# cvxgrp/qcqp

Hardware: AMD Instinct MI355X
Metric: restarts x coord-sweeps / sec (improve COORD_DESCENT phase-2 sweeps, 2n^2 flops each; whole step timed) (higher is better)
Workload: dtype f64

## Files before the change

### qcqp_amd/csrc/cd_life.hip

```cpp
#include "cd_life.h"

#include <cstdio>
#include <cstdlib>

#include "onevar.h"
#include "cd_phase1_sep.h"
#include "cd_chain.h"
#include "cd_roles.h"

namespace qcqpmi {
namespace {

constexpr int L2_WD = 1 << 21;
enum { L2_ABORT = 3 };

__device__ __attribute__((always_inline)) inline RqOwn l2_own(int NB, int CS, int m, int NMW) {
    RqOwn o;
    const int rest = NB - CS;
    o.NB = NB;
    if (m < 0) { o.first = rest; o.stride = 1; o.nu = CS; }
    else { o.first = m; o.stride = NMW; o.nu = m < rest ? (rest - m + NMW - 1) / NMW : 0; }
    return o;
}

// ... 982 lines not shown
                    if (l2_tl(sid, ct, TD)[cc] < 0) for (int64_t j = tid; j < n16; j += NT) Xg[j * 16 + cc] = 0.0;
                    continue;
                }
                if (!lf_generate) {
                    const int id = l2_tl(sid, ct, TD)[cc];
                    GLB const double *src = glb(a0.b.X) + ((int64_t)(id >> 4) * n16) * 16 + (id & 15);
                    for (int64_t j0 = tid; j0 < n16; j0 += 4 * NT) {
                        double t4[4];
#pragma unroll
                        for (int u = 0; u < 4; u++) t4[u] = (j0 + u * NT < n16) ? src[(j0 + u * NT) * 16] : 0.0;
#pragma unroll
                        for (int u = 0; u < 4; u++) if (j0 + u * NT < n16) Xg[(j0 + u * NT) * 16 + cc] = t4[u];
                    }
                }
            }
            if (lf_generate) {
                if (tid == 0) {
                    int cnt = 0;
                    for (int k = 0; k < NS; k++) if (l2_tl(snew, k >> 4, TD)[k & 15]) p1cols[cnt++] = k;
                    ctl[4] = cnt; ctl[5] = 0;
                }
                __syncthreads();
                const int ncolg = ctl[4], nchg = (int)((n16 + 127) / 128);
                for (;;) {
                    int ch = 0;
                    if (lane == 0) ch = atomicAdd(&ctl[5], 1);
                    ch = __builtin_amdgcn_readfirstlane(ch);
                    if (ch >= ncolg * nchg) break;
                    const int c = p1cols[ch / nchg], ct = c >> 4, cc = c & 15;
                    GLB double *Xg = Xg0 + (int64_t)ct * n16 * 16;
                    const int64_t j = (int64_t)(ch % nchg) * 128 + 2 * lane;
                    const uint64_t sd = l2_tl(sseed, ct, TD)[cc], gidx = l2_tl(sfirst, ct, TD)[cc] + (uint64_t)l2_tl(sid, ct, TD)[cc];
                    if (j < n16) {
                        double xo = 0.0;
                        const double xe = (j < P.n) ? keyed_normal_pair(sd, gidx, (uint64_t)j, &xo) : 0.0;
                        Xg[j * 16 + cc] = xe;
                        Xg[(j + 1) * 16 + cc] = (j + 1 < P.n) ? xo : 0.0;
                    }
                }
            }
            __syncthreads();
            if (lf->prof && tid == 0) atomicAdd((unsigned long long *)lf->prof + 4, (unsigned long long)((long long)__builtin_amdgcn_s_memtime() - pt0));
            if (lf_phase1) {
                const bool band2 = !MULTI && cq == 0.0 && rel == RELOP_EQ && cp > 1e-4 && cr < -1e-3;
                const int cw = band2 ? 128 : 64;
                const int nch = (int)((P.n + cw - 1) / cw);
                for (int64_t t = 0; t < a.num_iters; t++) {
                    if (tid == 0) {
                        int cnt = 0;
                        for (int k = 0; k < NS; k++) if (l2_tl(snew, k >> 4, TD)[k & 15] && !l2_tl(p1fin, k >> 4, TD)[k & 15]) p1cols[cnt++] = k;
                        ctl[4] = cnt; ctl[5] = 0;
                    }
                    if (tid < NS) { l2_tl(p1key, tid >> 4, TD)[tid & 15] = ordered_key(-QM_INF); l2_tl(p1upd, tid >> 4, TD)[tid & 15] = 0; }
                    __syncthreads();
                    const int ncol1 = ctl[4];
                    if (ncol1 == 0) break;
                    for (;;) {
                        int ch = 0;
                        if (lane == 0) ch = atomicAdd(&ctl[5], 1);
                        ch = __builtin_amdgcn_readfirstlane(ch);
                        if (ch >= ncol1 * nch) break;
                        const int c = p1cols[ch / nch], ct = c >> 4, cc = c & 15;
                        GLB double *Xg = Xg0 + (int64_t)ct * n16 * 16;
                        const uint64_t sd = l2_tl(sseed, ct, TD)[cc], gidx = l2_tl(sfirst, ct, TD)[cc] + (uint64_t)l2_tl(sid, ct, TD)[cc];
                        double va = -QM_INF;
                        int fl = 0;
                        if (band2) {
                            const int64_t i2[2] = {(int64_t)(ch % nch) * 128 + lane, (int64_t)(ch % nch) * 128 + 64 + lane};
                            const bool on2[2] = {i2[0] < P.n, i2[1] < P.n};
                            double x2[2] = {on2[0] ? Xg[i2[0] * 16 + cc] : 1.0, on2[1] ? Xg[i2[1] * 16 + cc] : 1.0};
                            P1Visit V2[2];
                            p1_band_visit_n<2>(cp, cq, cr, i2, x2, on2, a.tol, lf_viol_tol, sd, gidx, t, V2);
#pragma unroll
                            for (int k = 0; k < 2; k++)
                                if (on2[k]) {
                                    if (V2[k].moved) { Xg[i2[k] * 16 + cc] = x2[k]; fl |= 1; }
                                    if (V2[k].status) fl |= (-V2[k].status) << 8;
                                    va = V2[k].vafter > va ? V2[k].vafter : va;
                                }
                        } else {
                            const int64_t i = (int64_t)(ch % nch) * 64 + lane;
                            if (i < P.n) {
                                if (MULTI) {
                                    double xi = Xg[i * 16 + cc];
                                    P1Visit V;
                                    p1_sep_visit<MAXC>(P, i, xi, a.tol, lf_viol_tol, sd, gidx, t, V);
                                    fl = (V.moved ? 1 : 0) | ((-V.status) << 8);
                                    va = V.vafter;
                                    if (V.moved) Xg[i * 16 + cc] = xi;
                                } else {
                                    const double xi = p1_class_visit(cp, cq, cr, rel, i, Xg[i * 16 + cc], a.tol, lf_viol_tol, sd, gidx, t, &fl, &va);
                                    if (fl & 1) Xg[i * 16 + cc] = xi;
                                }
                            }
                        }
                        const double vmax = wave_max(va);
                        const bool anyupd = __builtin_amdgcn_ballot_w64((fl & 1) != 0) != 0ull;
                        const int st = (fl >> 8) ? -(fl >> 8) : 0;
                        if (lane == 0) { atomicMax(&l2_tl(p1key, ct, TD)[cc], ordered_key(vmax)); if (anyupd) l2_tl(p1upd, ct, TD)[cc] = 1; }
                        if (st) l2_tl(p1st, ct, TD)[cc] = st;
                    }
                    __syncthreads();
                    if (tid < NS && l2_tl(snew, tid >> 4, TD)[tid & 15] && !l2_tl(p1fin, tid >> 4, TD)[tid & 15]) {
                        const int st = tid >> 4, sc = tid & 15;
                        l2_tl(p1sw, st, TD)[sc]++;
                        if (ordered_unkey(l2_tl(p1key, st, TD)[sc]) < lf_viol_tol || !l2_tl(p1upd, st, TD)[sc]) l2_tl(p1fin, st, TD)[sc] = 1;
                    }
                    __syncthreads();
                }
            }
            if (lf->prof && tid == 0) atomicAdd((unsigned long long *)lf->prof + 17, (unsigned long long)((long long)__builtin_amdgcn_s_memtime() - pt0));
            if (tid < NS) l2_tl(p1key, tid >> 4, TD)[tid & 15] = ordered_key(-QM_INF);
            __syncthreads();
            for (int c = 0; c < NS; c++) {
                const int ct = c >> 4, cc = c & 15;
                if (lf_pre || !l2_tl(snew, ct, TD)[cc]) continue;
                GLB const double *Xg = Xg0 + (int64_t)ct * n16 * 16;
                double v = -QM_INF;
                for (int64_t i = tid; i < P.n; i += NT) {
                    const double x = Xg[i * 16 + cc];
                    if (MULTI) {
                        for (int e = P.cptr[i]; e < P.cptr[i + 1]; e++) {
                            const double f = (P.cp[e] * x + P.cq[e]) * x + P.cr[e];
                            const double w = viol_of(f, P.crel[e]);
                            v = w > v ? w : v;
                        }
                    } else {
                        const double f = (cp * x + cq) * x + cr;
                        const double w = (rel == RELOP_EQ) ? fabs(f) : (f > 0.0 ? f : 0.0);
                        v = w > v ? w : v;
                    }
                }
                v = wave_max(v);
                if (lane == 0) atomicMax(&l2_tl(p1key, ct, TD)[cc], ordered_key(v));
            }
            __syncthreads();
            if (tid < NS && l2_tl(snew, tid >> 4, TD)[tid & 15]) {
                const int st = tid >> 4, sc = tid & 15;
                double mvx;
                if (lf_pre) {
                    const int id = l2_tl(sid, st, TD)[sc];
                    mvx = glb(lf->preslack)[id];
                    l2_tl(p1sw, st, TD)[sc] = (int)glb(lf->sweeps1)[id];
                    l2_tl(p1st, st, TD)[sc] = glb(lf->status1)[id];
                    l2_tl(gatep, st, TD)[sc] = glb(lf->ran2)[id];
                } else {
                    mvx = ordered_unkey(l2_tl(p1key, st, TD)[sc]);
                    l2_tl(gatep, st, TD)[sc] = (mvx < lf_viol_tol && l2_tl(p1st, st, TD)[sc] == 0) ? 1 : 0;
                }
                l2_tl(slk, st, TD)[sc] = mvx;
                L2_STORE_SETS(st, sc, mvx)
            }
            __syncthreads();
            if (nlast < 16) {
                for (int w = tid; w < NS * (16 - nlast); w += NT) {
                    const int c = w % NS, ct = c >> 4, cc = c & 15, row = w / NS;
                    if (l2_tl(snew, ct, TD)[cc] || l2_tl(sid, ct, TD)[cc] < 0) {
                        const int nn = l2_tl(TC.n, ct, TD)[cc];
                        double xp = 0.0;
                        if (BK == L2_KIND_BAND) xp = nn >= 2 ? l2_tl(TC.lo, ct, TD)[16 * KCLV + cc] : 0.0;
                        else if (BK == L2_KIND_GEN) xp = nn >= 1 ? l2_tl(TC.hi, ct, TD)[cc] : 0.0;
                        else xp = nn >= 2 ? l2_tl(TC.hi, ct, TD)[16 * KCLV + cc] : l2_tl(TC.hi, ct, TD)[cc];
                        if (!(xp == xp) || __builtin_isinf(xp)) xp = 0.0;
                        (Xg0 + (int64_t)ct * n16 * 16)[(P.n + row) * 16 + cc] = xp;
                    }
                }
                __syncthreads();
            }
            if (LR) {
                const int r16 = 16 * a0.RB;
                const int y0n = lf_pre ? (int)lf->y0_count : 0;
                GLB const double *y0g = glb(lf->y0);
                for (int w = tid; w < NS * (32 + r16); w += NT) {
                    const int c = w % NS, ct = c >> 4, cc = c & 15, rowz = w / NS;
                    const int id = l2_tl(sid, ct, TD)[cc];
                    if (l2_tl(snew, ct, TD)[cc] || id < 0) {
                        double v = 0.0;
                        if (id >= 0 && id < y0n)
                            v = rowz < 32 ? (Xg0 + (int64_t)ct * n16 * 16)[(16 * (int64_t)(NB - 2) + rowz) * 16 + cc]
                                          : y0g[((int64_t)(id >> 4) * r16 + (rowz - 32)) * 16 + (id & 15)];
                        if (rowz < 32) l2_tl(pend, ct, TD)[rowz * 16 + cc] = v;
                        else l2_tl(ytile, ct, TD)[(rowz - 32) * 16 + cc] = v;
                    }
                }
                __syncthreads();
            }
            if (lf->prof && tid == 0) {
                int nn = 0;
                for (int k = 0; k < NS; k++) nn += l2_tl(snew, k >> 4, TD)[k & 15] ? 1 : 0;
                atomicAdd((unsigned long long *)lf->prof + 0, (unsigned long long)((long long)__builtin_amdgcn_s_memtime() - pt0));
                atomicAdd((unsigned long long *)lf->prof + 2, 1ull);
                atomicAdd((unsigned long long *)lf->prof + 3, (unsigned long long)nn);
            }
            __builtin_amdgcn_s_setprio(0);
        }
        if (role == 0) {
            long long *cs_ = l2_tl(cst, rtile, TD);
            if (l2_tl(snew, rtile, TD)[r]) {
#pragma unroll
                for (int f = 0; f < 6; f++) cs_[f * 64 + lane] = 0;
                const int pass = l2_tl(gatep, rtile, TD)[r];
                bool load = LR != 0;
                if (LR) {
                    GLB const CdLife *lf = glb(lifep);
                    if (lf->prebuilt && l2_tl(sid, rtile, TD)[r] < (int)lf->y0_count) load = false;
                }
                cs_[6 * 64 + lane] = 0;
                cs_[4 * 64 + lane] = (pass && !PRE && !load) ? 0 : 1;
                cs_[7 * 64 + lane] = (pass ? (PRE ? 4 : 0) : 1) | (load ? 8 : 0);
                cs_[8 * 64 + lane] = 0;
            } else if (l2_tl(sid, rtile, TD)[r] < 0) {
                cs_[4 * 64 + lane] = 1; cs_[6 * 64 + lane] = 0;
                cs_[7 * 64 + lane] = 2; cs_[8 * 64 + lane] = 0;
            }
        }
        __syncthreads();
        if (tid == 0 && glb(lifep)->prof) *(long long *)(ctl + 6) = (long long)__builtin_amdgcn_s_memtime();

        if (role > 0) {
            if (LR) l2_mfma_lr_role<NMW>(role - 1, rtile);
            else l2_mfma_role<NMW, CS>(role - 1, rtile);
        } else l2_chain_role<NMW, CS, KIND, TILES, LR>(rtile);

        __syncthreads();
        if (sy[L2_ABORT] || (TILES > 1 && l2_tl((int *)sy, 1, TD)[L2_ABORT])) {
            if (tid == 0) __hip_atomic_store(glb(a0.abort), 1, __ATOMIC_RELAXED, __HIP_MEMORY_SCOPE_AGENT);
            break;
        }
        if (tid == 0 && glb(lifep)->prof)
        {
            const long long now_ = (long long)__builtin_amdgcn_s_memtime();
            atomicAdd((unsigned long long *)glb(lifep)->prof + 5, (unsigned long long)(now_ - *(long long *)(ctl + 6)));
            atomicAdd((unsigned long long *)glb(lifep)->prof + 20, (unsigned long long)(now_ - *(long long *)(ctl + 8)));
        }
        {
            const int e0 = P.cptr[P.krep[0]];
            const double cp = P.cp[e0], cq = P.cq[e0], cr = P.cr[e0];
            const int rel = P.crel[e0];
            if (tid == 0) { int cnt = 0; for (int k = 0; k < NS; k++) if (l2_tl(sfin, k >> 4, TD)[k & 15]) p1cols[cnt++] = k; ctl[4] = cnt; }
            if (tid < NS) l2_tl(p1key, tid >> 4, TD)[tid & 15] = ordered_key(-QM_INF);
            __syncthreads();
            const int nfin = ctl[4];
            const int64_t items = (int64_t)nfin * n16;
            for (int64_t w0 = tid; w0 < items; w0 += (int64_t)NT * 8) {
                double xv8[8];
#pragma unroll
                for (int u = 0; u < 8; u++) {
                    const int64_t w = w0 + (int64_t)NT * u;
                    const int col = p1cols[w < items ? w / n16 : 0];
                    const int64_t i = w % n16;
                    xv8[u] = (w < items && i < P.n) ? (Xg0 + (int64_t)(col >> 4) * n16 * 16)[i * 16 + (col & 15)] : 0.0;
                }
#pragma unroll
                for (int u = 0; u < 8; u++) {
                    const int64_t w = w0 + (int64_t)NT * u;
                    if (w < items) {
                        const int col = p1cols[w / n16], id = l2_tl(sid, col >> 4, TD)[col & 15];
                        const int64_t i = w % n16;
                        glb(a0.b.X)[((int64_t)(id >> 4) * n16 + i) * 16 + (id & 15)] = xv8[u];
                        if (i < P.n) {
                            if (MULTI) {
                                double vv = -QM_INF;
                                for (int e = P.cptr[i]; e < P.cptr[i + 1]; e++) {
                                    const double w_ = viol_of((P.cp[e] * xv8[u] + P.cq[e]) * xv8[u] + P.cr[e], P.crel[e]);
                                    vv = w_ > vv ? w_ : vv;
                                }
                                atomicMax(&l2_tl(p1key, col >> 4, TD)[col & 15], ordered_key(vv));
                            } else {
                                const double f = (cp * xv8[u] + cq) * xv8[u] + cr;
                                const double vv = (rel == RELOP_EQ) ? fabs(f) : (f > 0.0 ? f : 0.0);
                                atomicMax(&l2_tl(p1key, col >> 4, TD)[col & 15], ordered_key(vv));
                            }
                        }
                    }
                }
            }
            __syncthreads();
            if (tid < NS && l2_tl(sfin, tid >> 4, TD)[tid & 15]) {
                const int st = tid >> 4, sc = tid & 15;
                const double mx = ordered_unkey(l2_tl(p1key, st, TD)[sc]);
                const int id = l2_tl(sid, st, TD)[sc];
                glb(a0.b.visits)[id] = l2_tl(ovis, st, TD)[sc]; glb(a0.b.accepted)[id] = l2_tl(oacc, st, TD)[sc]; glb(a0.b.sweeps)[id] = l2_tl(oswp, st, TD)[sc];
                glb(a0.b.status)[id] = l2_tl(ost, st, TD)[sc];
                if (a0.b.f0out) glb(a0.b.f0out)[id] = l2_tl(of0, st, TD)[sc];
                if (a0.b.mvout) glb(a0.b.mvout)[id] = mx;
                GLB const CdLife *lf = glb(lifep);
                glb(lf->sweeps1)[id] = l2_tl(p1sw, st, TD)[sc]; glb(lf->status1)[id] = l2_tl(p1st, st, TD)[sc];
                glb(lf->ran2)[id] = (uint8_t)l2_tl(gatep, st, TD)[sc];
                l2_tl(sid, st, TD)[sc] = -1; l2_tl(sfin, st, TD)[sc] = 0;
            }
            __syncthreads();
        }
    }
    if (tid0 == 0 && lf0->prof) {
        const unsigned long long dtl = (unsigned long long)((long long)__builtin_amdgcn_s_memtime() - life_t0);
        atomicAdd((unsigned long long *)lf0->prof + 1, dtl);
        atomicMax((unsigned long long *)lf0->prof + 16, dtl);
    }
}

#undef L2_STORE_SETS

constexpr int L2P_NT = 256;
__global__ __launch_bounds__(L2P_NT) void cd_life_prep_kernel(DevProblem P, const CdLife *life, double *X, int64_t num_iters, double tol) {
    __shared__ unsigned long long key[16];
    __shared__ int upd[16], st1[16], fin[16], sw[16], nact;
    const int tid = threadIdx.x, s = tid & 15, g = tid >> 4;
    GLB const CdLife *lf = glb(life);
    const int64_t id = (int64_t)blockIdx.x * 16 + s;
    const bool valid = id < lf->Rtotal;
    const int64_t n = P.n, n16 = P.n16;
    GLB double *Xt = glb(X) + (int64_t)blockIdx.x * n16 * 16 + s;
    const double viol_tol = lf->viol_tol;
    uint64_t sd = 0, gidx = 0;
    if (valid) {
        const uint64_t pop = (uint64_t)id / (uint64_t)lf->Rpop, rho = (uint64_t)id % (uint64_t)lf->Rpop;
        sd = lf->seed + pop * lf->seed_stride;
        gidx = lf->first_index + pop * lf->first_stride + rho;
    }
    if (lf->generate && valid) {
        for (int64_t j = 2 * g; j < n16; j += 32) {
            double xo = 0.0;
            const double xe = (j < n) ? keyed_normal_pair(sd, gidx, (uint64_t)j, &xo) : 0.0;
            Xt[16 * j] = xe;
            Xt[16 * (j + 1)] = (j + 1 < n) ? xo : 0.0;
        }
    }
    const int e0 = P.cptr[P.krep[0]];
    const double cp = P.cp[e0], cq = P.cq[e0], cr = P.cr[e0];
    const int rel = P.crel[e0];
    if (tid < 16) { fin[tid] = valid ? 0 : 1; sw[tid] = 0; st1[tid] = 0; }
    if (lf->phase1) {
        const bool band2 = cq == 0.0 && rel == RELOP_EQ && cp > 1e-4 && cr < -1e-3;
        for (int64_t t = 0; t < num_iters; t++) {
            if (tid < 16) { key[tid] = ordered_key(-QM_INF); upd[tid] = 0; }
            __syncthreads();
            if (tid == 0) { int c = 0; for (int k = 0; k < 16; k++) c += fin[k] ? 0 : 1; nact = c; }
            __syncthreads();
            if (nact == 0) break;
            double va = -QM_INF;
            int moved = 0, stv = 0;
            if (!fin[s]) {
                for (int64_t j = 2 * g; j < n; j += 32) {
                    if (band2) {
                        const int64_t i2[2] = {j, j + 1};
                        const bool on2[2] = {true, j + 1 < n};
                        double x2[2] = {Xt[16 * j], on2[1] ? Xt[16 * (j + 1)] : 1.0};
                        P1Visit V2[2];
                        p1_band_visit_n<2>(cp, cq, cr, i2, x2, on2, tol, viol_tol, sd, gidx, t, V2);
#pragma unroll
                        for (int k = 0; k < 2; k++)
                            if (on2[k]) {
                                if (V2[k].moved) { Xt[16 * i2[k]] = x2[k]; moved = 1; }
                                if (V2[k].status) stv = V2[k].status;
                                va = V2[k].vafter > va ? V2[k].vafter : va;
                            }
                    } else {
                        for (int64_t i = j; i < j + 2 && i < n; i++) {
                            int fl = 0;
                            double v = 0.0;
                            const double xi = p1_class_visit(cp, cq, cr, rel, i, Xt[16 * i], tol, viol_tol, sd, gidx, t, &fl, &v);
                            if (fl & 1) { Xt[16 * i] = xi; moved = 1; }
                            if (fl >> 8) stv = -(fl >> 8);
                            va = v > va ? v : va;
                        }
                    }
                }
            }
#pragma unroll
            for (int o = 16; o <= 32; o <<= 1) {
                const double w = __shfl_xor(va, o, 64);
                va = w > va ? w : va;
                moved |= __shfl_xor(moved, o, 64);
            }
            if ((tid & 63) < 16 && !fin[s]) { atomicMax(&key[s], ordered_key(va)); if (moved) upd[s] = 1; }
            if (stv) st1[s] = stv;
            __syncthreads();
            if (tid < 16 && !fin[tid]) {
                sw[tid]++;
                if (ordered_unkey(key[tid]) < viol_tol || !upd[tid]) fin[tid] = 1;
            }
        }
    }
    __syncthreads();
    if (tid < 16) key[tid] = ordered_key(-QM_INF);
    __syncthreads();
    double v = -QM_INF;
    if (valid)
        for (int64_t j = 2 * g; j < n; j += 32)
            for (int64_t i = j; i < j + 2 && i < n; i++) {
                const double x = Xt[16 * i];
                const double f = (cp * x + cq) * x + cr;
                const double w = (rel == RELOP_EQ) ? fabs(f) : (f > 0.0 ? f : 0.0);
                v = w > v ? w : v;
            }
#pragma unroll
    for (int o = 16; o <= 32; o <<= 1) { const double w = __shfl_xor(v, o, 64); v = w > v ? w : v; }
    if ((tid & 63) < 16 && valid) atomicMax(&key[s], ordered_key(v));
    __syncthreads();
    if (tid < 16 && valid) {
        const double mvx = ordered_unkey(key[tid]);
        glb(const_cast<double *>(lf->preslack))[id] = mvx;
        glb(lf->sweeps1)[id] = sw[tid];
        glb(lf->status1)[id] = st1[tid];
        glb(lf->ran2)[id] = (mvx < viol_tol && st1[tid] == 0) ? 1 : 0;
    }
}

constexpr int L2Y_NT = 256, L2Y_BW = 4, L2Y_TW = 4;
__global__ __launch_bounds__(L2Y_NT, 2) void cd_life_y0_kernel(const double *__restrict__ X, const double *__restrict__ Upack, double *__restrict__ Y0,
                                                               int NB, int RB, int ntiles, int64_t n16) {
    const int lane = threadIdx.x & 63;
    const int wave = __builtin_amdgcn_readfirstlane((int)(threadIdx.x >> 6));
    const int nbg = (RB + L2Y_BW - 1) / L2Y_BW;
    const int64_t gw = (int64_t)blockIdx.x * (L2Y_NT / 64) + wave;
    const int beta0 = (int)(gw % nbg) * L2Y_BW;
    const int64_t t0 = gw / nbg * L2Y_TW;
    if (t0 >= ntiles) return;
    GLB const v2d_ *ua[L2Y_BW];
    GLB const double *xt[L2Y_TW];
#pragma unroll
    for (int u = 0; u < L2Y_BW; u++) ua[u] = (GLB const v2d_ *)glb(Upack) + (int64_t)(beta0 + u < RB ? beta0 + u : RB - 1) * 128 + lane;
#pragma unroll
    for (int k = 0; k < L2Y_TW; k++) xt[k] = glb(X) + (t0 + k < ntiles ? t0 + k : (int64_t)ntiles - 1) * n16 * 16 + lane;
    v4d_ y[L2Y_BW][L2Y_TW];
#pragma unroll
    for (int u = 0; u < L2Y_BW; u++)
#pragma unroll
        for (int k = 0; k < L2Y_TW; k++) y[u][k] = v4d_{0.0, 0.0, 0.0, 0.0};
    const int nblk = NB - 2;
    v2d_ a[L2Y_BW][2];
    double x[L2Y_TW][4];
#pragma unroll
    for (int u = 0; u < L2Y_BW; u++) { a[u][0] = ua[u][0]; a[u][1] = ua[u][64]; }
#pragma unroll
    for (int k = 0; k < L2Y_TW; k++)
#pragma unroll
        for (int v = 0; v < 4; v++) x[k][v] = xt[k][v * 64];
    for (int b = 0; b < nblk; b++) {
        const int bn = b + 1 < nblk ? b + 1 : b;
        v2d_ an[L2Y_BW][2];
        double xn[L2Y_TW][4];
#pragma unroll
        for (int u = 0; u < L2Y_BW; u++) { an[u][0] = ua[u][(int64_t)bn * RB * 128]; an[u][1] = ua[u][(int64_t)bn * RB * 128 + 64]; }
#pragma unroll
        for (int k = 0; k < L2Y_TW; k++)
#pragma unroll
            for (int v = 0; v < 4; v++) xn[k][v] = xt[k][(int64_t)bn * 256 + v * 64];
#pragma unroll
        for (int v = 0; v < 4; v++)
#pragma unroll
            for (int u = 0; u < L2Y_BW; u++)
#pragma unroll
                for (int k = 0; k < L2Y_TW; k++) y[u][k] = __builtin_amdgcn_mfma_f64_16x16x4f64(a[u][v >> 1][v & 1], x[k][v], y[u][k], 0, 0, 0);
#pragma unroll
        for (int u = 0; u < L2Y_BW; u++) { a[u][0] = an[u][0]; a[u][1] = an[u][1]; }
#pragma unroll
        for (int k = 0; k < L2Y_TW; k++)
#pragma unroll
            for (int v = 0; v < 4; v++) x[k][v] = xn[k][v];
    }
    const int64_t r16 = 16 * (int64_t)RB;
#pragma unroll
    for (int u = 0; u < L2Y_BW; u++)
#pragma unroll
        for (int k = 0; k < L2Y_TW; k++)
            if (beta0 + u < RB && t0 + k < ntiles) {
                GLB double *dst = glb(Y0) + ((t0 + k) * r16 + 16 * (beta0 + u)) * 16 + lane;
#pragma unroll
                for (int v = 0; v < 4; v++) dst[v * 64] = y[u][k][v];
            }
}

__global__ void l2_pack_kernel(DevProblem P, double *Dpack, double *Spack) {
    const int b = blockIdx.x, t = threadIdx.x;
    const int64_t n16 = P.n16;
    const int rr = t >> 4, cc = t & 15;
    Dpack[(int64_t)b * 256 + t] = (cc > rr) ? P.P0[(16 * (int64_t)b + rr) * n16 + 16 * b + cc] : 0.0;
    if (t < 16) {
        const int64_t i = 16 * (int64_t)b + t;
        const double d = P.P0[i * n16 + i], rc = P.rcp2d[i];
        Spack[(int64_t)b * 48 + t] = 0.5 * P.q0[i];
        Spack[(int64_t)b * 48 + 16 + t] = rc + rc;
        Spack[(int64_t)b * 48 + 32 + t] = d;
    }
}

__global__ void l2_pack_factor_kernel(const double *__restrict__ L, double *__restrict__ Gpack, double *__restrict__ Upack, int NB, int RB) {
    const int64_t idx = (int64_t)blockIdx.x * blockDim.x + threadIdx.x;
    if (idx >= (int64_t)NB * RB * 256) return;
    const int e = (int)(idx & 1), lane = (int)((idx >> 1) & 63), vp = (int)((idx >> 7) & 1);
    const int64_t rest = idx >> 8;
    const int beta = (int)(rest % RB), b = (int)(rest / RB), v = 2 * vp + e;
    const int64_t r16 = 16 * (int64_t)RB;
    Gpack[idx] = L[(16 * (int64_t)b + (lane & 15)) * r16 + 16 * beta + 4 * v + (lane >> 4)];
    Upack[idx] = L[(16 * (int64_t)b + 4 * v + (lane >> 4)) * r16 + 16 * beta + (lane & 15)];
}

template <int NMW, int CS, int TILES, int LR>
int l2_launch_kind(const CdLife2Args &a, int kind, int wgs, size_t lds, hipStream_t st) {
    constexpr bool MK = TILES == 1 && !LR;
    if (!MK && (kind == L2_KIND_GENK || kind == L2_KIND_LINK)) return (int)hipErrorInvalidValue;
    if (LR && kind == L2_KIND_SGN) return (int)hipErrorInvalidValue;
    auto k = kind == L2_KIND_SGN ? cd_life_kernel<NMW, CS, LR ? L2_KIND_GEN : L2_KIND_SGN, TILES, LR> : kind == L2_KIND_BAND ? cd_life_kernel<NMW, CS, L2_KIND_BAND, TILES, LR> : (kind == L2_KIND_GEN || LR) ? cd_life_kernel<NMW, CS, L2_KIND_GEN, TILES, LR>
             : kind == L2_KIND_GENK ? cd_life_kernel<NMW, CS, MK ? L2_KIND_GENK : L2_KIND_GEN, TILES, LR>
             : kind == L2_KIND_LINK ? cd_life_kernel<NMW, CS, MK ? L2_KIND_LINK : L2_KIND_GEN, TILES, LR>
                                    : cd_life_kernel<NMW, CS, LR ? L2_KIND_GEN : L2_KIND_LIN, TILES, LR>;
    hipError_t e = hipFuncSetAttribute((const void *)k, hipFuncAttributeMaxDynamicSharedMemorySize, (int)lds);
    if (e != hipSuccess) return (int)e;
    hipLaunchKernelGGL(k, dim3((unsigned)wgs), dim3((NMW == 3 && TILES == 1) ? 256 : 512), lds, st, a);
    return (int)hipGetLastError();
}

}

size_t cd_life2_lds_bytes(int nmw, int cs, int tiles, int lr, int kind) {
    const bool multi = kind == L2_KIND_GENK || kind == L2_KIND_LINK;
    return ((size_t)L2_SHARED_DOUBLES + (size_t)tiles * (size_t)l2_tile_doubles(nmw, cs > 0 ? cs : 1, lr, multi ? L2_KCL : 1, multi ? 2 : 1)) * sizeof(double) + 256;
}

bool cd_life2_factor_ok(const DevProblem &P, int64_t r) {
    const int64_t r16 = (r + 15) / 16 * 16;
    if (r < 1 || r16 > 16 * L2_YBMAX || P.NB < 8) return false;
    return true;
}

int cd_life2_pack_factor(const double *Lrow, double *Gpack, double *Upack, int NB, int RB, hipStream_t st) {
    const int64_t tot = (int64_t)NB * RB * 256;
    hipLaunchKernelGGL(l2_pack_factor_kernel, dim3((unsigned)((tot + 255) / 256)), dim3(256), 0, st, Lrow, Gpack, Upack, NB, RB);
    return (int)hipGetLastError();
}

int cd_life2_prep_launch(const DevProblem &P, const CdLife *life, double *X, int64_t Rtotal, int64_t num_iters, double tol, hipStream_t st) {
    hipLaunchKernelGGL(cd_life_prep_kernel, dim3((unsigned)((Rtotal + 15) / 16)), dim3(L2P_NT), 0, st, P, life, X, num_iters, tol);
    return (int)hipGetLastError();
}

int cd_life2_y0_launch(const double *X, const double *Upack, double *Y0, int NB, int RB, int64_t n16, int64_t count, hipStream_t st) {
    if (count < 1) return (int)hipSuccess;
    if (NB < 3 || RB < 1) return (int)hipErrorInvalidValue;
    const int64_t ntiles = (count + 15) / 16;
    const int64_t waves = (ntiles + L2Y_TW - 1) / L2Y_TW * ((RB + L2Y_BW - 1) / L2Y_BW);
    hipLaunchKernelGGL(cd_life_y0_kernel, dim3((unsigned)((waves + L2Y_NT / 64 - 1) / (L2Y_NT / 64))), dim3(L2Y_NT), 0, st, X, Upack, Y0, NB, RB, (int)ntiles, n16);
    return (int)hipGetLastError();
}

int cd_life2_max_wgs(int nmw, int cus, int tiles) { return (nmw == 3 && tiles == 1) ? 2 * cus : cus; }

bool cd_life2_config(const DevProblem &P, int Kreal, int objclass, bool symcls, int factor_rb, int *nmw, int *cs, int *kind) {
    if (!P.sep || P.maxc < 1 || P.maxc > 2 || Kreal < 1 || Kreal > L2_KCL) return false;
    const bool multi = P.maxc > 1 || Kreal > 1;
    if (objclass != 0 && objclass != 1 && objclass != 2) return false;
    if (objclass == 0 && multi) return false;
    const int NB = (int)P.NB;
    if (NB < 3) return false;
    int w, c;
    if (NB <= 4) { w = 3; c = 0; }
    else if (NB - 4 <= 3 * RQ_MAXU) { w = 3; c = (NB < 8) ? 2 : 4; }
    else if (factor_rb > 0 && !multi && objclass == 1 && NB <= 256) { w = 3; c = 0; }
    else if (NB - 4 <= 7 * RQ_MAXU) { w = 7; c = 4; }
    else return false;
    *nmw = w; *cs = c;
    *kind = objclass == 0 ? L2_KIND_SGN : multi ? (objclass == 2 ? L2_KIND_LINK : L2_KIND_GENK) : objclass == 2 ? L2_KIND_LIN : (symcls ? L2_KIND_BAND : L2_KIND_GEN);
    return true;
}

int cd_life2_tiles(const DevProblem &P, int nmw, int cs, int64_t restarts, int cus, int requested, int lr) {
    (void)P; (void)restarts; (void)cus;
    if (!lr || nmw != 3 || cs != 0) return 1;
    int t = requested;
    if (const char *ev = getenv("QCQPMI_L2_TILES")) t = atoi(ev);
    return t == 2 ? 2 : 1;
}

int cd_life2_pack(const DevProblem &P, double *Dpack, double *Spack, hipStream_t st) {
    hipLaunchKernelGGL(l2_pack_kernel, dim3((unsigned)P.NB), dim3(256), 0, st, P, Dpack, Spack);
    return (int)hipGetLastError();
}

int cd_life2_launch(const CdLife2Args &a, int nmw, int cs, int kind, int tiles, int wgs, hipStream_t st) {
    const int lr = a.RB > 0 ? 1 : 0;
    if (const char *ev = getenv("QCQPMI_L2_CS")) {
        const int k2 = atoi(ev);
        if (!lr && nmw == 3 && tiles == 1 && (k2 == 0 || k2 == 2 || k2 == 4) && k2 + 3 <= (int)a.P.NB && (int)a.P.NB - k2 <= 3 * RQ_MAXU) cs = k2;
    }
    const size_t lds = cd_life2_lds_bytes(nmw, cs, tiles, lr, kind);
    if (getenv("QCQPMI_L2_DEBUG")) {
        int occ = -1;
        hipError_t e = lr ? (tiles == 2 ? hipOccupancyMaxActiveBlocksPerMultiprocessor(&occ, cd_life_kernel<3, 0, L2_KIND_BAND, 2, 1>, 512, lds)
                                        : hipOccupancyMaxActiveBlocksPerMultiprocessor(&occ, cd_life_kernel<3, 0, L2_KIND_BAND, 1, 1>, 256, lds))
                     : nmw == 3 ? hipOccupancyMaxActiveBlocksPerMultiprocessor(&occ, cd_life_kernel<3, 4, L2_KIND_BAND, 1, 0>, 256, lds)
                                : hipOccupancyMaxActiveBlocksPerMultiprocessor(&occ, cd_life_kernel<7, 4, L2_KIND_BAND, 1, 0>, 512, lds);
        fprintf(stderr, "cd_life2_launch: nmw %d cs %d kind %d tiles %d lr %d wgs %d lds %zu: occupancy %d workgroups per CU (%s)\n", nmw, cs, kind, tiles, lr, wgs, lds, occ, hipGetErrorString(e));
    }
    if (wgs < 1) wgs = 1;
    if (lr) {
        if (nmw != 3 || cs != 0 || kind == L2_KIND_LIN || kind == L2_KIND_SGN) return (int)hipErrorInvalidValue;
        return tiles == 2 ? l2_launch_kind<3, 0, 2, 1>(a, kind, wgs, lds, st) : l2_launch_kind<3, 0, 1, 1>(a, kind, wgs, lds, st);
    }
    if (tiles != 1) return (int)hipErrorInvalidValue;
    if (nmw == 3) {
        if (cs == 0) return l2_launch_kind<3, 0, 1, 0>(a, kind, wgs, lds, st);
        if (cs == 2) return l2_launch_kind<3, 2, 1, 0>(a, kind, wgs, lds, st);
        if (cs == 4) return l2_launch_kind<3, 4, 1, 0>(a, kind, wgs, lds, st);
        return (int)hipErrorInvalidValue;
    }
    if (nmw == 7 && cs == 4) return l2_launch_kind<7, 4, 1, 0>(a, kind, wgs, lds, st);
    return (int)hipErrorInvalidValue;
}

const char *cd_life2_name(int nmw, int kind, int tiles, int lr) {
    if (kind == L2_KIND_GENK) return nmw == 3 ? "cd_life_kernel<3,gen,classes>" : "cd_life_kernel<7,gen,classes>";
    if (kind == L2_KIND_LINK) return nmw == 3 ? "cd_life_kernel<3,lin,classes>" : "cd_life_kernel<7,lin,classes>";
    if (kind == L2_KIND_SGN) return nmw == 3 ? "cd_life_kernel<3,sgn>" : "cd_life_kernel<7,sgn>";
    if (lr) return tiles == 2 ? (kind == L2_KIND_BAND ? "cd_life_kernel<3,band,2 tiles,factored>" : "cd_life_kernel<3,gen,2 tiles,factored>")
                              : (kind == L2_KIND_BAND ? "cd_life_kernel<3,band,factored>" : "cd_life_kernel<3,gen,factored>");
    if (tiles == 2) return kind == L2_KIND_BAND ? "cd_life_kernel<3,band,2 tiles>" : kind == L2_KIND_GEN ? "cd_life_kernel<3,gen,2 tiles>" : "cd_life_kernel<3,lin,2 tiles>";
    if (nmw == 3) return kind == L2_KIND_BAND ? "cd_life_kernel<3,band>" : kind == L2_KIND_GEN ? "cd_life_kernel<3,gen>" : "cd_life_kernel<3,lin>";
    return kind == L2_KIND_BAND ? "cd_life_kernel<7,band>" : kind == L2_KIND_GEN ? "cd_life_kernel<7,gen>" : "cd_life_kernel<7,lin>";
}

}
```

### qcqp_amd/csrc/cd_phase1_sep.h

```cpp
#pragma once
#include "kernels.h"
#include "onevar.h"

namespace qcqpmi {

__device__ inline double viol_of(double f, int relop) {
    if (relop == RELOP_EQ) return fabs(f);
    return f > 0.0 ? f : 0.0;
}

struct P1Visit {
    bool visited;
    bool moved;
    double vafter;
    int status;
};

template <int MAXC>
__device__ inline void p1_sep_visit_core(int mf, const double (&cp)[MAXC], const double (&cq)[MAXC], const double (&cr)[MAXC],
                                         const int (&crel)[MAXC], int64_t i, double &xi, double tol, double viol_tol, uint64_t seed,
                                         uint64_t grestart, int64_t t, P1Visit &V) {
    V.visited = true; V.moved = false; V.vafter = -QM_INF; V.status = 0;
    double viol = -QM_INF;
#pragma unroll
    for (int k = 0; k < MAXC; k++)
        if (k < mf) {
            double v = viol_of(xi * (cp[k] * xi + cq[k]) + cr[k], crel[k]);
            viol = v > viol ? v : viol;
        }
    double new_xi = xi, new_viol = viol;
    double ss = -tol, es = viol - viol_tol;
    uint32_t it = 0;
    FeasSet<MAXC> Cp;
    uint32_t itp = 0;
    bool pending = false;
    const bool band = mf == 1 && cq[0] == 0.0 && crel[0] == RELOP_EQ && cp[0] > 1e-4;
    double sp = 0.0;
    while (es - ss > tol) {
        double s = (ss + es) / 2.0;
        if (band) {
            const uint32_t itb = it++;
            const double D1 = 0.0 - 4.0 * cp[0] * (cr[0] - s);
            const double D2 = 0.0 - 4.0 * (-cp[0]) * (-cr[0] - s);
            const bool nonempty = D1 > 0.0 && (D2 < 0.0 || D2 < D1);
            if (!nonempty) { ss = s; continue; }
            sp = s; itp = itb; pending = true;
            new_viol = s; es = s;
            continue;
        }
        FeasSet<MAXC> C;
        if (mf == 1) feasible_set_single<MAXC>(cp[0], cq[0], cr[0], crel[0], s, C);
        else feasible_set<MAXC>(cp, cq, cr, crel, mf, s, C);
        const uint32_t itc = it++;
        if (C.n == 0) { ss = s; continue; }
        bool unb = false;
#pragma unroll
        for (int j = 0; j <= MAXC; j++) unb = unb || (j < C.n && (__builtin_isinf(C.lo[j]) || __builtin_isinf(C.hi[j])));
        if (unb) {
            DrawKey dk{seed, grestart, (uint32_t)i, (uint32_t)t, itc};
            double xn;
            int got = onevar_minimise<MAXC>(0.0, 0.0, 0.0, C, dk, &xn);
            if (got < 0) { V.status = got; pending = false; break; }
            new_xi = xn; pending = false;
        } else {
            Cp = C; itp = itc; pending = true;
        }
        new_viol = s; es = s;
    }
    if (pending && band) feasible_set_single<MAXC>(cp[0], cq[0], cr[0], crel[0], sp, Cp);
    if (pending) {
        DrawKey dk{seed, grestart, (uint32_t)i, (uint32_t)t, itp};
        double xn = xi;
        const int got = onevar_minimise<MAXC>(0.0, 0.0, 0.0, Cp, dk, &xn);
        if (got == 1) new_xi = xn;
        else { new_viol = viol; if (got < 0) V.status = got; }
    }
    if (new_viol < viol) { xi = new_xi; V.moved = true; }
#pragma unroll
    for (int k = 0; k < MAXC; k++)
        if (k < mf) {
            double v = viol_of((cp[k] * xi + cq[k]) * xi + cr[k], crel[k]);
            V.vafter = v > V.vafter ? v : V.vafter;
        }
}

__device__ inline void p1_band_visit(double p, double q, double r, int64_t i, double &xi, double tol, double viol_tol, uint64_t seed,
                                     uint64_t grestart, int64_t t, P1Visit &V) {
    V.visited = true; V.moved = false; V.status = 0;
    const double viol = fabs(xi * (p * xi + q) + r);
    double new_xi = xi, new_viol = viol;
    double ss = -tol, es = viol - viol_tol, sp = 0.0;
    uint32_t it = 0, itp = 0;
    bool pending = false;
    const bool plain = r < -1e-3;
    const double guard = 1e-9 * (1.0 - r);
    if (plain) {
        while (es - ss > tol) {
            const double s = (ss + es) / 2.0;
            const uint32_t itb = it++;
            bool nonempty = s > 0.0;
            if (__builtin_expect(!(fabs(s) > guard), 0)) {
                const double D1 = 0.0 - 4.0 * p * (r - s);
                const double D2 = 0.0 - 4.0 * (-p) * (-r - s);
                nonempty = D1 > 0.0 && (D2 < 0.0 || D2 < D1);
            }
            ss = nonempty ? ss : s;
            es = nonempty ? s : es;
            sp = nonempty ? s : sp;
            itp = nonempty ? itb : itp;
            pending = pending || nonempty;
        }
        if (pending) new_viol = sp;
    } else {
        while (es - ss > tol) {
            const double s = (ss + es) / 2.0;
            const uint32_t itb = it++;
            const double D1 = 0.0 - 4.0 * p * (r - s);
            const double D2 = 0.0 - 4.0 * (-p) * (-r - s);
            const bool nonempty = D1 > 0.0 && (D2 < 0.0 || D2 < D1);
            if (!nonempty) { ss = s; continue; }
            sp = s; itp = itb; pending = true;
            new_viol = s; es = s;
        }
    }
    if (pending) {
        const double r1 = r - sp, r2 = -r - sp;
        const double rsA = r1 - 0.0, rsB = r2 - 0.0;
        const double DA = q * q - 4.0 * p * rsA;
        const bool hasA = DA >= 0.0;
        const double rDA = sqrt(hasA ? DA : 0.0);
        const double pB = -p, qB = -q;
        const double DB = qB * qB - 4.0 * pB * rsB;
        const bool twoB = DB >= 0.0;
        const double rDB = sqrt(twoB ? DB : 0.0);
        const double tA = rDA / (2.0 * p), tB = rDB / (2.0 * p);
        const double alo = -tA, ahi = tA;
        const double bhi0 = twoB ? -tB : QM_INF;
        const double blo1 = tB;
        const double l0 = alo > -QM_INF ? alo : -QM_INF, h0 = ahi < bhi0 ? ahi : bhi0;
        const bool ok0 = hasA && l0 <= h0;
        const double l1 = alo > blo1 ? alo : blo1, h1 = ahi < QM_INF ? ahi : QM_INF;
        const bool ok1 = hasA && twoB && l1 <= h1;
        int n = (ok0 ? 1 : 0) + (ok1 ? 1 : 0);
        double lo0 = ok0 ? l0 : (ok1 ? l1 : 0.0), hi0 = ok0 ? h0 : (ok1 ? h1 : 0.0);
        double lo1 = (ok0 && ok1) ? l1 : 0.0, hi1 = (ok0 && ok1) ? h1 : 0.0;
        if (n == 2 && lo0 == lo1 && hi0 == hi1) n = 0;
        else if (n == 2 && hi0 == lo1) { hi0 = hi1; n = 1; }
        else if (n == 2 && hi1 == lo0) { lo0 = lo1; n = 1; }
        const bool k0 = n >= 1 && lo0 != hi0 && hi0 != QM_INF;
        const bool k1 = n >= 2 && lo1 != hi1 && hi1 != QM_INF;
        if (k0 && k1 && lo1 < lo0) {
            double tt;
            tt = lo0; lo0 = lo1; lo1 = tt;
            tt = hi0; hi0 = hi1; hi1 = tt;
        }
        const int cn = (k0 ? 1 : 0) + (k1 ? 1 : 0);
        const double c0lo = k0 ? lo0 : lo1, c0hi = k0 ? hi0 : hi1;
        int got = 0;
        double xn = xi;
        if (cn > 0) {
            const U4 rnd = cd_draw(seed, grestart, (uint32_t)i, (uint32_t)t, itp);
            const int c = draw_choice(rnd, cn);
            const double lo = (c == 1) ? lo1 : c0lo, hi = (c == 1) ? hi1 : c0hi;
            if (__builtin_isinf(lo) || __builtin_isinf(hi)) got = -1;
            else { xn = draw_uniform(rnd, lo, hi); got = 1; }
        }
        if (got == 1) new_xi = xn;
        else { new_viol = viol; if (got < 0) V.status = got; }
    }
    if (new_viol < viol) { xi = new_xi; V.moved = true; }
    V.vafter = fabs((p * xi + q) * xi + r);
}

template <int NV>
__device__ inline void p1_band_visit_n(double p, double q, double r, const int64_t (&i)[NV], double (&xi)[NV], const bool (&on)[NV], double tol,
                                       double viol_tol, uint64_t seed, uint64_t grestart, int64_t t, P1Visit (&V)[NV]) {
    double viol[NV], ss[NV], es[NV], sp[NV];
    uint32_t it[NV], itp[NV];
    bool pending[NV];
    const double guard = 1e-9 * (1.0 - r);
#pragma unroll
    for (int k = 0; k < NV; k++) {
        V[k].visited = true; V[k].moved = false; V[k].status = 0;
        viol[k] = fabs(xi[k] * (p * xi[k] + q) + r);
        ss[k] = -tol; es[k] = on[k] ? viol[k] - viol_tol : -tol; sp[k] = 0.0;
        it[k] = 0; itp[k] = 0; pending[k] = false;
    }
    for (;;) {
        bool any = false;
#pragma unroll
        for (int k = 0; k < NV; k++) any = any || (es[k] - ss[k] > tol);
        if (!any) break;
#pragma unroll
        for (int k = 0; k < NV; k++) {
            const bool act = es[k] - ss[k] > tol;
            const double s = (ss[k] + es[k]) / 2.0;
            const uint32_t itb = it[k];
            it[k] += act ? 1u : 0u;
            bool nonempty = s > 0.0;
            if (__builtin_expect(act && !(fabs(s) > guard), 0)) {
                const double D1 = 0.0 - 4.0 * p * (r - s);
                const double D2 = 0.0 - 4.0 * (-p) * (-r - s);
                nonempty = D1 > 0.0 && (D2 < 0.0 || D2 < D1);
            }
            const bool up = act && nonempty, dn = act && !nonempty;
            ss[k] = dn ? s : ss[k];
            es[k] = up ? s : es[k];
            sp[k] = up ? s : sp[k];
            itp[k] = up ? itb : itp[k];
            pending[k] = pending[k] || up;
        }
    }
#pragma unroll
    for (int k = 0; k < NV; k++) {
        const double spk = sp[k];
        const double r1 = r - spk, r2 = -r - spk;
        const double rsA = r1 - 0.0, rsB = r2 - 0.0;
        const double DA = q * q - 4.0 * p * rsA;
        const bool hasA = DA >= 0.0;
        const double rDA = sqrt(hasA ? DA : 0.0);
        const double pB = -p, qB = -q;
        const double DB = qB * qB - 4.0 * pB * rsB;
        const bool twoB = DB >= 0.0;
        const double rDB = sqrt(twoB ? DB : 0.0);
        const double tA = rDA / (2.0 * p), tB = rDB / (2.0 * p);
        const double alo = -tA, ahi = tA;
        const double bhi0 = twoB ? -tB : QM_INF;
        const double blo1 = tB;
        const double l0 = alo > -QM_INF ? alo : -QM_INF, h0 = ahi < bhi0 ? ahi : bhi0;
        const bool ok0 = hasA && l0 <= h0;
        const double l1 = alo > blo1 ? alo : blo1, h1 = ahi < QM_INF ? ahi : QM_INF;
        const bool ok1 = hasA && twoB && l1 <= h1;
        int n = (ok0 ? 1 : 0) + (ok1 ? 1 : 0);
        double lo0 = ok0 ? l0 : (ok1 ? l1 : 0.0), hi0 = ok0 ? h0 : (ok1 ? h1 : 0.0);
        double lo1 = (ok0 && ok1) ? l1 : 0.0, hi1 = (ok0 && ok1) ? h1 : 0.0;
        const bool same = n == 2 && lo0 == lo1 && hi0 == hi1;
        const bool m01 = !same && n == 2 && hi0 == lo1;
        const bool m10 = !same && !m01 && n == 2 && hi1 == lo0;
        hi0 = m01 ? hi1 : hi0;
        lo0 = m10 ? lo1 : lo0;
        n = same ? 0 : ((m01 || m10) ? 1 : n);
        const bool k0 = n >= 1 && lo0 != hi0 && hi0 != QM_INF;
        const bool k1 = n >= 2 && lo1 != hi1 && hi1 != QM_INF;
        const bool sw = k0 && k1 && lo1 < lo0;
        const double a0 = sw ? lo1 : lo0, b0 = sw ? hi1 : hi0, a1 = sw ? lo0 : lo1, b1 = sw ? hi0 : hi1;
        const int cn = (k0 ? 1 : 0) + (k1 ? 1 : 0);
        const double c0lo = k0 ? a0 : a1, c0hi = k0 ? b0 : b1;
        const U4 rnd = cd_draw(seed, grestart, (uint32_t)i[k], (uint32_t)t, itp[k]);
        const int c = draw_choice(rnd, cn);
        const double lo = (c == 1) ? a1 : c0lo, hi = (c == 1) ? b1 : c0hi;
        const bool unb = __builtin_isinf(lo) || __builtin_isinf(hi);
        const double xn = draw_uniform(rnd, lo, hi);
        const int got = (cn > 0) ? (unb ? -1 : 1) : 0;
        double new_xi = xi[k], new_viol = viol[k];
        if (pending[k]) {
            if (got == 1) { new_xi = xn; new_viol = spk; }
            else if (got < 0) V[k].status = got;
        }
        if (on[k] && new_viol < viol[k]) { xi[k] = new_xi; V[k].moved = true; }
        V[k].vafter = fabs((p * xi[k] + q) * xi[k] + r);
    }
}

__device__ __attribute__((always_inline)) inline double p1_class_visit(double p, double q, double r, int relop, int64_t i, double x, double tol,
                                                                        double viol_tol, uint64_t seed, uint64_t restart, int64_t t, int *flags,
                                                                        double *vafter) {
    P1Visit V;
    if (q == 0.0 && relop == RELOP_EQ && p > 1e-4) {
        p1_band_visit(p, q, r, i, x, tol, viol_tol, seed, restart, t, V);
    } else {
        const double cp[1] = {p}, cq[1] = {q}, cr[1] = {r};
        const int crel[1] = {relop};
        p1_sep_visit_core<1>(1, cp, cq, cr, crel, i, x, tol, viol_tol, seed, restart, t, V);
    }
    *flags = (V.moved ? 1 : 0) | ((-V.status) << 8);
    *vafter = V.vafter;
    return x;
}

template <int MAXC>
__device__ inline void p1_sep_visit(const DevProblem &P, int64_t i, double &xi, double tol, double viol_tol, uint64_t seed,
                                    uint64_t grestart, int64_t t, P1Visit &V) {
    V.visited = false; V.moved = false; V.vafter = -QM_INF; V.status = 0;
    const int e0 = P.cptr[i], mf = P.cptr[i + 1] - e0;
    if (mf == 0) { V.status = -3; return; }
    double cp[MAXC], cq[MAXC], cr[MAXC];
    int crel[MAXC];
#pragma unroll
    for (int k = 0; k < MAXC; k++) {
        bool ok = k < mf;
        cp[k] = ok ? P.cp[e0 + k] : 0.0; cq[k] = ok ? P.cq[e0 + k] : 0.0;
        cr[k] = ok ? P.cr[e0 + k] : 0.0; crel[k] = ok ? P.crel[e0 + k] : RELOP_LE;
    }
    p1_sep_visit_core<MAXC>(mf, cp, cq, cr, crel, i, xi, tol, viol_tol, seed, grestart, t, V);
}

}
```

Baseline: 28.65 million.

## Compact active restarts in phase-1 prep kernel and add fast bisection phase

In the prep kernel's phase-1 loop, once some of the 16 restarts in a block have finished, the block now spreads all 256 threads over each remaining restart in turn instead of leaving lanes of finished restarts idle. It adds extra shuffle reductions for the compacted mode. It also adds a fast first phase to the band bisection that halves the interval while the midpoint is clearly positive, skipping the guard test in that stretch. Launch bounds now request 3 blocks per CU, which may limit registers.

```diff
diff --git a/qcqp_amd/csrc/cd_life.hip b/qcqp_amd/csrc/cd_life.hip
--- a/qcqp_amd/csrc/cd_life.hip
+++ b/qcqp_amd/csrc/cd_life.hip
@@ -1308,9 +1308,9 @@
 #undef L2_STORE_SETS
 
 constexpr int L2P_NT = 256;
-__global__ __launch_bounds__(L2P_NT) void cd_life_prep_kernel(DevProblem P, const CdLife *life, double *X, int64_t num_iters, double tol) {
-    __shared__ unsigned long long key[16];
-    __shared__ int upd[16], st1[16], fin[16], sw[16], nact;
+__global__ __launch_bounds__(L2P_NT, 3) void cd_life_prep_kernel(DevProblem P, const CdLife *life, double *X, int64_t num_iters, double tol) {
+    __shared__ unsigned long long key[16], csd[16], cgi[16];
+    __shared__ int upd[16], st1[16], fin[16], sw[16], cols[16], nact;
     const int tid = threadIdx.x, s = tid & 15, g = tid >> 4;
     GLB const CdLife *lf = glb(life);
     const int64_t id = (int64_t)blockIdx.x * 16 + s;
@@ -1335,52 +1335,70 @@
     const int e0 = P.cptr[P.krep[0]];
     const double cp = P.cp[e0], cq = P.cq[e0], cr = P.cr[e0];
     const int rel = P.crel[e0];
-    if (tid < 16) { fin[tid] = valid ? 0 : 1; sw[tid] = 0; st1[tid] = 0; }
+    if (tid < 16) { fin[tid] = valid ? 0 : 1; sw[tid] = 0; st1[tid] = 0; csd[tid] = sd; cgi[tid] = gidx; }
     if (lf->phase1) {
         const bool band2 = cq == 0.0 && rel == RELOP_EQ && cp > 1e-4 && cr < -1e-3;
+        GLB double *Xtile = glb(X) + (int64_t)blockIdx.x * n16 * 16;
         for (int64_t t = 0; t < num_iters; t++) {
             if (tid < 16) { key[tid] = ordered_key(-QM_INF); upd[tid] = 0; }
             __syncthreads();
-            if (tid == 0) { int c = 0; for (int k = 0; k < 16; k++) c += fin[k] ? 0 : 1; nact = c; }
+            if (tid == 0) { int c = 0; for (int k = 0; k < 16; k++) if (!fin[k]) cols[c++] = k; nact = c; }
             __syncthreads();
             if (nact == 0) break;
-            double va = -QM_INF;
-            int moved = 0, stv = 0;
-            if (!fin[s]) {
-                for (int64_t j = 2 * g; j < n; j += 32) {
-                    if (band2) {
-                        const int64_t i2[2] = {j, j + 1};
-                        const bool on2[2] = {true, j + 1 < n};
-                        double x2[2] = {Xt[16 * j], on2[1] ? Xt[16 * (j + 1)] : 1.0};
-                        P1Visit V2[2];
-                        p1_band_visit_n<2>(cp, cq, cr, i2, x2, on2, tol, viol_tol, sd, gidx, t, V2);
-#pragma unroll
-                        for (int k = 0; k < 2; k++)
-                            if (on2[k]) {
-                                if (V2[k].moved) { Xt[16 * i2[k]] = x2[k]; moved = 1; }
-                                if (V2[k].status) stv = V2[k].status;
-                                va = V2[k].vafter > va ? V2[k].vafter : va;
+            const bool compact = t > 0 && nact < 16;
+            const int npass = compact ? nact : 1;
+            const int64_t j0 = compact ? 2 * tid : 2 * g, jstep = compact ? 2 * L2P_NT : 32;
+            for (int qq = 0; qq < npass; qq++) {
+                const int c = compact ? cols[qq] : s;
+                const bool live = compact || !fin[s];
+                GLB double *Xc = Xtile + c;
+                const uint64_t sdc = csd[c], gic = cgi[c];
+                double va = -QM_INF;
+                int moved = 0, stv = 0;
+                if (live) {
+                    for (int64_t j = j0; j < n; j += jstep) {
+                        if (band2) {
+                            const int64_t i2[2] = {j, j + 1};
+                            const bool on2[2] = {true, j + 1 < n};
+                            double x2[2] = {Xc[16 * j], on2[1] ? Xc[16 * (j + 1)] : 1.0};
+                            P1Visit V2[2];
+                            p1_band_visit_n<2, true>(cp, cq, cr, i2, x2, on2, tol, viol_tol, sdc, gic, t, V2);
+#pragma unroll
+                            for (int k = 0; k < 2; k++)
+                                if (on2[k]) {
+                                    if (V2[k].moved) { Xc[16 * i2[k]] = x2[k]; moved = 1; }
+                                    if (V2[k].status) stv = V2[k].status;
+                                    va = V2[k].vafter > va ? V2[k].vafter : va;
+                                }
+                        } else {
+                            for (int64_t i = j; i < j + 2 && i < n; i++) {
+                                int fl = 0;
+                                double v = 0.0;
+                                const double xi = p1_class_visit(cp, cq, cr, rel, i, Xc[16 * i], tol, viol_tol, sdc, gic, t, &fl, &v);
+                                if (fl & 1) { Xc[16 * i] = xi; moved = 1; }
+                                if (fl >> 8) stv = -(fl >> 8);
+                                va = v > va ? v : va;
                             }
-                    } else {
-                        for (int64_t i = j; i < j + 2 && i < n; i++) {
-                            int fl = 0;
-                            double v = 0.0;
-                            const double xi = p1_class_visit(cp, cq, cr, rel, i, Xt[16 * i], tol, viol_tol, sd, gidx, t, &fl, &v);
-                            if (fl & 1) { Xt[16 * i] = xi; moved = 1; }
-                            if (fl >> 8) stv = -(fl >> 8);
-                            va = v > va ? v : va;
                         }
                     }
                 }
-            }
-#pragma unroll
-            for (int o = 16; o <= 32; o <<= 1) {
-                const double w = __shfl_xor(va, o, 64);
-                va = w > va ? w : va;
-                moved |= __shfl_xor(moved, o, 64);
-            }
-            if ((tid & 63) < 16 && !fin[s]) { atomicMax(&key[s], ordered_key(va)); if (moved) upd[s] = 1; }
-            if (stv) st1[s] = stv;
+#pragma unroll
+                for (int o = 16; o <= 32; o <<= 1) {
+                    const double w = __shfl_xor(va, o, 64);
+                    va = w > va ? w : va;
+                    moved |= __shfl_xor(moved, o, 64);
+                }
+                if (compact) {
+#pragma unroll
+                    for (int o = 1; o <= 8; o <<= 1) {
+                        const double w = __shfl_xor(va, o, 64);
+                        va = w > va ? w : va;
+                        moved |= __shfl_xor(moved, o, 64);
+                    }
+                }
+                if ((tid & 63) < (compact ? 1 : 16) && live) { atomicMax(&key[c], ordered_key(va)); if (moved) upd[c] = 1; }
+                if (stv) st1[c] = stv;
+            }
             __syncthreads();
             if (tid < 16 && !fin[tid]) {
                 sw[tid]++;
diff --git a/qcqp_amd/csrc/cd_phase1_sep.h b/qcqp_amd/csrc/cd_phase1_sep.h
--- a/qcqp_amd/csrc/cd_phase1_sep.h
+++ b/qcqp_amd/csrc/cd_phase1_sep.h
@@ -1,6 +1,7 @@
 #pragma once
 #include "kernels.h"
 #include "onevar.h"
+#include "p1_bisect.h"
 
 namespace qcqpmi {
 
@@ -172,7 +173,7 @@
     V.vafter = fabs((p * xi + q) * xi + r);
 }
 
-template <int NV>
+template <int NV, bool FASTA = false>
 __device__ inline void p1_band_visit_n(double p, double q, double r, const int64_t (&i)[NV], double (&xi)[NV], const bool (&on)[NV], double tol,
                                        double viol_tol, uint64_t seed, uint64_t grestart, int64_t t, P1Visit (&V)[NV]) {
     double viol[NV], ss[NV], es[NV], sp[NV];
@@ -186,29 +187,33 @@
         ss[k] = -tol; es[k] = on[k] ? viol[k] - viol_tol : -tol; sp[k] = 0.0;
         it[k] = 0; itp[k] = 0; pending[k] = false;
     }
-    for (;;) {
-        bool any = false;
-#pragma unroll
-        for (int k = 0; k < NV; k++) any = any || (es[k] - ss[k] > tol);
-        if (!any) break;
-#pragma unroll
-        for (int k = 0; k < NV; k++) {
-            const bool act = es[k] - ss[k] > tol;
-            const double s = (ss[k] + es[k]) / 2.0;
-            const uint32_t itb = it[k];
-            it[k] += act ? 1u : 0u;
-            bool nonempty = s > 0.0;
-            if (__builtin_expect(act && !(fabs(s) > guard), 0)) {
-                const double D1 = 0.0 - 4.0 * p * (r - s);
-                const double D2 = 0.0 - 4.0 * (-p) * (-r - s);
-                nonempty = D1 > 0.0 && (D2 < 0.0 || D2 < D1);
+    if constexpr (FASTA) {
+        p1_band_bisect<NV>(p, r, tol, ss, es, sp, it, itp, pending);
+    } else {
+        for (;;) {
+            bool any = false;
+#pragma unroll
+            for (int k = 0; k < NV; k++) any = any || (es[k] - ss[k] > tol);
+            if (!any) break;
+#pragma unroll
+            for (int k = 0; k < NV; k++) {
+                const bool act = es[k] - ss[k] > tol;
+                const double s = (ss[k] + es[k]) / 2.0;
+                const uint32_t itb = it[k];
+                it[k] += act ? 1u : 0u;
+                bool nonempty = s > 0.0;
+                if (__builtin_expect(act && !(fabs(s) > guard), 0)) {
+                    const double D1 = 0.0 - 4.0 * p * (r - s);
+                    const double D2 = 0.0 - 4.0 * (-p) * (-r - s);
+                    nonempty = D1 > 0.0 && (D2 < 0.0 || D2 < D1);
+                }
+                const bool up = act && nonempty, dn = act && !nonempty;
+                ss[k] = dn ? s : ss[k];
+                es[k] = up ? s : es[k];
+                sp[k] = up ? s : sp[k];
+                itp[k] = up ? itb : itp[k];
+                pending[k] = pending[k] || up;
             }
-            const bool up = act && nonempty, dn = act && !nonempty;
-            ss[k] = dn ? s : ss[k];
-            es[k] = up ? s : es[k];
-            sp[k] = up ? s : sp[k];
-            itp[k] = up ? itb : itp[k];
-            pending[k] = pending[k] || up;
         }
     }
 #pragma unroll
diff --git a/qcqp_amd/csrc/p1_bisect.h b/qcqp_amd/csrc/p1_bisect.h
--- /dev/null
+++ b/qcqp_amd/csrc/p1_bisect.h
@@ -0,0 +1,84 @@
+#pragma once
+#include <stdint.h>
+
+#ifndef QCQPMI_P1_FASTBISECT
+#define QCQPMI_P1_FASTBISECT 1
+#endif
+
+#if defined(__HIPCC__)
+#define P1B_FN __host__ __device__ inline
+#else
+#define P1B_FN inline
+#endif
+
+namespace qcqpmi {
+
+template <int NV>
+P1B_FN void p1_band_bisect_general(double p, double r, double tol, double guard, double (&ss)[NV], double (&es)[NV], double (&sp)[NV],
+                                   uint32_t (&it)[NV], uint32_t (&itp)[NV], bool (&pending)[NV]) {
+    for (;;) {
+        bool any = false;
+#pragma unroll
+        for (int k = 0; k < NV; k++) any = any || (es[k] - ss[k] > tol);
+        if (!any) break;
+#pragma unroll
+        for (int k = 0; k < NV; k++) {
+            const bool act = es[k] - ss[k] > tol;
+            const double s = (ss[k] + es[k]) / 2.0;
+            const uint32_t itb = it[k];
+            it[k] += act ? 1u : 0u;
+            bool nonempty = s > 0.0;
+            if (__builtin_expect(act && !(__builtin_fabs(s) > guard), 0)) {
+                const double D1 = 0.0 - 4.0 * p * (r - s);
+                const double D2 = 0.0 - 4.0 * (-p) * (-r - s);
+                nonempty = D1 > 0.0 && (D2 < 0.0 || D2 < D1);
+            }
+            const bool up = act && nonempty, dn = act && !nonempty;
+            ss[k] = dn ? s : ss[k];
+            es[k] = up ? s : es[k];
+            sp[k] = up ? s : sp[k];
+            itp[k] = up ? itb : itp[k];
+            pending[k] = pending[k] || up;
+        }
+    }
+}
+
+template <int NV>
+P1B_FN void p1_band_bisect_phase_a(double tol, double guard, const double (&ss)[NV], double (&es)[NV], double (&sp)[NV], uint32_t (&it)[NV],
+                                   uint32_t (&itp)[NV], bool (&pending)[NV]) {
+    uint32_t na[NV];
+#pragma unroll
+    for (int k = 0; k < NV; k++) na[k] = 0;
+    for (;;) {
+        bool any = false;
+        bool go[NV];
+        double s[NV];
+#pragma unroll
+        for (int k = 0; k < NV; k++) {
+            s[k] = (ss[k] + es[k]) / 2.0;
+            go[k] = es[k] - ss[k] > tol && s[k] > guard;
+            any = any || go[k];
+        }
+        if (!any) break;
+#pragma unroll
+        for (int k = 0; k < NV; k++) {
+            es[k] = go[k] ? s[k] : es[k];
+            na[k] += go[k] ? 1u : 0u;
+        }
+    }
+#pragma unroll
+    for (int k = 0; k < NV; k++)
+        if (na[k]) { sp[k] = es[k]; itp[k] = it[k] + na[k] - 1u; it[k] += na[k]; pending[k] = true; }
+}
+
+template <int NV>
+P1B_FN void p1_band_bisect(double p, double r, double tol, double (&ss)[NV], double (&es)[NV], double (&sp)[NV], uint32_t (&it)[NV],
+                           uint32_t (&itp)[NV], bool (&pending)[NV]) {
+    const double guard = 1e-9 * (1.0 - r);
+#if QCQPMI_P1_FASTBISECT
+    p1_band_bisect_phase_a<NV>(tol, guard, ss, es, sp, it, itp, pending);
+#endif
+    p1_band_bisect_general<NV>(p, r, tol, guard, ss, es, sp, it, itp, pending);
+}
+
+}
```

Result: faster. 29.19 million, median of 6 (+1.9%).
